# h3poteto/aws-global-accelerator-controller

Hardware: NVIDIA H100
Metric: objects reconciled/sec at 10^6 Service+Ingress; change-set bit-exact vs Go ref (higher is better)
Workload: dtype u8/u32 (bytes and indices)

## Files before the change

aws-global-accelerator-controller_b200/csrc/gar_pipeline.h:

```cpp
#pragma once

#include <stdio.h>
#include <stdlib.h>

#include <initializer_list>

#include "gar_rows.h"

#if defined(__CUDA_ARCH__)
#define GAR_ATOMIC_ADD(p, v) atomicAdd((p), (v))
#else
#define GAR_ATOMIC_ADD(p, v) (*(p) += (v))
#endif


enum Slot {
  S_DERIVED, S_OFLAGS, S_OKEY_HASH, S_STAGE_GA, S_STAGE_R53, S_ANN_R53, S_ANN_NAME, S_ANN_TAGS, S_ANN_LISTEN, S_DPORT_BEGIN, S_DPORTS,
  S_TOK_CODE, S_TOK_NAME, S_TOK_REGION,
  S_ACC_FLAGS, S_ACC_OWNER_KEY, S_ACC_OWNER, S_ACC_THOST, S_ACC_MANAGED, S_ACC_OWNER_HASH, S_ACC_THOST_HASH, S_REC_NAME_HASH, S_VAL_KEY_HASH,
  S_REC_ZONE, S_VAL_REC, S_VAL_CLS, S_VAL_KEY, S_VAL_ORPHAN, S_VAL_LINK, S_ACC_DIGEST,
  S_R53_MODE, S_R53_ACC, S_R53_ACC_DNS, S_PAIR_BEGIN, S_PAIR_OBJ, S_PAIR_HN, S_PAIR_CODE, S_PAIR_ZONE, S_PAIR_REC,
  S_IX_LB, S_IX_OWNER = S_IX_LB + 3, S_IX_THOST = S_IX_OWNER + 3, S_IX_ZONE = S_IX_THOST + 3, S_IX_VAL = S_IX_ZONE + 3,
  S_IX_ALIAS = S_IX_VAL + 3, S_IX_OBJ = S_IX_ALIAS + 3, S_IX_OVN = S_IX_OBJ + 3,
  S_SORT_KEYS = S_IX_OVN + 3, S_SORT_VALS, S_SORT_KEYS_ALT, S_SORT_VALS_ALT, S_SORT_TAGS,
  S_COUNTS, S_STATUS_GA, S_STATUS_R53, S_OPS, S_ERRFLAG, S_IX_EG, S_IX_EG_ENT, S_IX_EG_PAD,
  S_VAL_OBJ, S_ACC_OBJ, S_OBJ_CANON, S_OWN_BEGIN, S_OWN_FILL, S_OWN_ENT, S_OWN_MULTI,
  S_IXA_BEGIN, S_IXA_FILL, S_IXA_ENT, S_IXA_MULTI, S_OVN_FILL, S_OVN_MULTI, S_LB_HASH, S_REC_FLAGS, S_LBI_RES,
  S_NSLOTS
};


struct FClassify {
  DevTables T;
  Work W;
  u32 *derived_public;
  u8 *oflags;
  u32 *errflag;
  GAR_HD void operator()(u32 i) const {
    classify_object(T, W, i);
    W.obj_canon[i] = i;
    u32 dv = W.derived[i];
    if (dv & OBJ_KEY_BAD) GAR_ATOMIC_ADD(errflag, 1u);
    derived_public[i] = dv & 0xFFu;
  }
};
struct FTokenise {
  DevTables T;
  Work W;
  static constexpr int kStageCols = 1;
  static constexpr u32 kStageBytes = 24 * 1024;
  static constexpr bool kStageByDefault = true;
  GAR_HD void operator()(u32 i) const { tokenise_hostname(T, W, i); }
  GAR_HD const u8 *stage_slab(int) const { return T.o.slab; }
  GAR_HD bool stage_window(int, u32 r0, u32 r1, u64 *lo, u64 *hi) const {
    gar_str a = T.o.lbi_hostname[r0], b = T.o.lbi_hostname[r1 - 1];
    *lo = GAR_STR_OFF(a);
    *hi = GAR_STR_OFF(b) + GAR_STR_LEN(b);
    return true;
  }
  template <class View>
  GAR_HD void run(u32 i, const View &view) const { tokenise_hostname_at(T, W, i, view(0, T.o.lbi_hostname[i])); }
};
struct FDigestAccel {
  DevTables T;
  Work W;
  GAR_HD void operator()(u32 i) const { digest_accelerator(T, W, i); }
};
struct FExpand {
  const u32 *begin;
  u32 nparents;
  u32 *parent_of;
  GAR_HD void operator()(u32 c) const {
    u32 lo = 0, hi = nparents;
    while (hi - lo > 1) {
      u32 mid = (lo + hi) >> 1;
      if (begin[mid] <= c) lo = mid;
      else hi = mid;
    }
    parent_of[c] = lo;
  }
// ... 58 lines not shown
  }
};
constexpr u32 BIG_BLOCKS = 528;
struct FClassifyBigRecords {
  DevTables T;
  Work W;
  const u32 *big, *huge;
  GAR_HD void operator()(u32 i) const {
    const u32 blk = i >> 8, tid = i & 255u, nbig = big[0], nhuge = huge[0];
    for (u32 k = blk; k < nbig; k += BIG_BLOCKS) {
      u32 r = big[1 + k];
      for (u32 v = T.a.rec_val_begin[r] + tid; v < T.a.rec_val_begin[r + 1]; v += 256) {
        W.val_rec[v] = r;
        classify_value(T, W, v);
      }
    }
    for (u32 k = 0; k < nhuge; k++) {
      u32 r = huge[1 + k];
      for (u32 v = T.a.rec_val_begin[r] + i; v < T.a.rec_val_begin[r + 1]; v += BIG_BLOCKS * 256) {
        W.val_rec[v] = r;
        classify_value(T, W, v);
      }
    }
  }
};
struct FJsonCount {
  DevTables T;
  Work W;
  GAR_HD void operator()(u32 i) const {
    u32 n = 0;
    if (W.derived[i] & GAR_DV_PORTS_FROM_ANN) {
      u32 stk[GAR_JSON_STACK_WORDS];
      int c = json_listen_ports(mkstr(T.o.slab, W.ann_listen[i]), nullptr, stk);
      n = c < 0 ? 0u : (u32)c;
    }
    W.dport_begin[i] = n;
  }
};
struct FJsonWrite {
  DevTables T;
  Work W;
  GAR_HD void operator()(u32 i) const {
    if (!(W.derived[i] & GAR_DV_PORTS_FROM_ANN)) return;
    if (W.dport_begin[i + 1] == W.dport_begin[i] || W.dport_begin[i + 1] > W.dport_cap) return;
    u32 stk[GAR_JSON_STACK_WORDS];
    json_listen_ports(mkstr(T.o.slab, W.ann_listen[i]), W.dports + W.dport_begin[i], stk);
  }
};

struct FLbHash {
  DevTables T;
  Work W;
  GAR_HD void operator()(u32 i) const {
    u64 h = key_hash_lb(mkstr(T.a.slab, T.a.lb_region[i]), mkstr(T.a.slab, T.a.lb_name[i]));
    W.lb_hash[i] = h;
    ix_count(W.hist[IX_LB], h);
  }
};
struct FRowLb {
  DevTables T;
  Work W;
  GAR_HD bool make(u32 i, u64 *h, IdxEntry *e) const {
    *h = W.lb_hash[i];
    e->a0 = T.a.lb_state[i];
    e->a1 = 0;
    e->s0 = T.a.lb_name[i];
    e->s1 = T.a.lb_region[i];
    return true;
  }
};
struct FRowOwner {
  DevTables T;
  Work W;
  GAR_HD bool make(u32 i, u64 *h, IdxEntry *e) const {
    u32 fl = W.acc_flags[i];
    *h = W.acc_owner_hash[i];
    e->a0 = fl;
    e->a1 = 0;
    e->s0 = W.acc_owner_key[i];
    e->s1 = 0;
    return (fl & ACC_MINE) && (fl & ACC_OWNER_KEYED) && i < W.acc_guest_from;
  }
};
struct FRowThost {
  DevTables T;
  Work W;
  GAR_HD bool make(u32 i, u64 *h, IdxEntry *e) const {
    *h = W.acc_thost_hash[i];
    e->a0 = e->a1 = 0;
    e->s0 = W.acc_thost[i];
    e->s1 = T.a.acc_dns[i];
    return (W.acc_flags[i] & ACC_MINE) != 0 && (!W.sharded || i >= W.acc_guest_from);
  }
};
struct FRowZone {
  DevTables T;
  GAR_HD bool make(u32 i, u64 *h, IdxEntry *e) const {
    Str zn = mkstr(T.a.slab, T.a.zone_name[i]);
    bool valid = zn.n >= 1 && zn.p[zn.n - 1] == '.';
    *h = valid ? key_hash_str(substr(zn, 0, zn.n - 1)) : 0;
    e->a0 = e->a1 = 0;
    e->s0 = T.a.zone_name[i];
    e->s1 = 0;
    return valid;
  }
};
struct FZoneLenMask {
  DevTables T;
  Work W;
  unsigned long long *mask;
  GAR_HD void operator()(u32 z) const {
    Str zn = mkstr(T.a.slab, T.a.zone_name[z]);
    if (zn.n < 1 || zn.p[zn.n - 1] != '.') return;
    ix_count(W.hist[IX_ZONE], key_hash_str(substr(zn, 0, zn.n - 1)));
    u32 b = zn.n - 1 < 255 ? zn.n - 1 : 255;
#if defined(__CUDA_ARCH__)
    atomicOr(&mask[b >> 6], 1ull << (b & 63));
#else
    mask[b >> 6] |= 1ull << (b & 63);
#endif
// ... 596 lines not shown
    return HashIdx{begin, ent, nb - 1};
  }

  bool prepared = false;
  u64 n_dports = 0;
  u32 *errflag = nullptr;

  u32 acc_guest_from = 0xFFFFFFFFu;
  u32 sharded = 0;
  bool orphan_sweep = true;
  bool allow_empty_cache = false;

  void alloc_obj_work() {
    const u32 n = T.o.n_objects, nlbi = T.o.n_lbi;
    W.derived = (u32 *)be.ensure(S_DERIVED, 4 * (size_t)(n + 1));
    W.okey_hash = (u64 *)be.ensure(S_OKEY_HASH, 8 * (size_t)(n + 1));
    W.ann_r53 = (gar_str *)be.ensure(S_ANN_R53, 8 * (size_t)(n + 1));
    W.ann_name = (gar_str *)be.ensure(S_ANN_NAME, 8 * (size_t)(n + 1));
    W.ann_tags = (gar_str *)be.ensure(S_ANN_TAGS, 8 * (size_t)(n + 1));
    W.ann_listen = (gar_str *)be.ensure(S_ANN_LISTEN, 8 * (size_t)(n + 1));
    W.dport_begin = (u32 *)be.out_dport_begin(n);
    W.tok_code = (u8 *)be.out_tok_code(nlbi);
    W.tok_name = (gar_str *)be.out_tok_name(nlbi);
    W.tok_region = (gar_str *)be.out_tok_region(nlbi);
    W.lbi_res = (LbiRes *)be.ensure(S_LBI_RES, sizeof(LbiRes) * (size_t)(nlbi + 1));
    W.r53_mode = (u8 *)be.ensure(S_R53_MODE, (size_t)n + 1);
    W.r53_acc = (u32 *)be.ensure(S_R53_ACC, 4 * (size_t)(n + 1));
    W.r53_acc_dns = (gar_str *)be.ensure(S_R53_ACC_DNS, 8 * (size_t)(n + 1));
    W.obj_canon = (u32 *)be.ensure(S_OBJ_CANON, 4 * (size_t)(n + 1));
  }
  CanonHook canon_hook(u32 b0, u32 b1) const { return CanonHook{W.obj_canon, T.o.slab, b0, b1}; }
  void alloc_work() {
    const u32 nacc = T.a.n_accels, nrec = T.a.n_records, nval = T.a.n_values;
    alloc_obj_work();
    W.acc_flags = (u32 *)be.ensure(S_ACC_FLAGS, 4 * (size_t)(nacc + 1));
    W.acc_owner_key = (gar_str *)be.ensure(S_ACC_OWNER_KEY, 8 * (size_t)(nacc + 1));
    W.acc_owner = (gar_str *)be.ensure(S_ACC_OWNER, 8 * (size_t)(nacc + 1));
    W.acc_thost = (gar_str *)be.ensure(S_ACC_THOST, 8 * (size_t)(nacc + 1));
    W.acc_managed = (gar_str *)be.ensure(S_ACC_MANAGED, 8 * (size_t)(nacc + 1));
    W.acc_owner_hash = (u64 *)be.ensure(S_ACC_OWNER_HASH, 8 * (size_t)(nacc + 1));
    W.acc_thost_hash = (u64 *)be.ensure(S_ACC_THOST_HASH, 8 * (size_t)(nacc + 1));
    W.rec_name_hash = (u64 *)be.ensure(S_REC_NAME_HASH, 8 * (size_t)(nrec + 1));
    W.val_key_hash = (u64 *)be.ensure(S_VAL_KEY_HASH, 8 * (size_t)(nval + 1));
    W.rec_zone = (u32 *)be.ensure(S_REC_ZONE, 4 * (size_t)(nrec + 1));
    W.val_rec = (u32 *)be.ensure(S_VAL_REC, 4 * (size_t)(nval + 1));
    W.val_cls = (u8 *)be.ensure(S_VAL_CLS, nval + 1);
    W.val_key = (gar_str *)be.ensure(S_VAL_KEY, 8 * (size_t)(nval + 1));
    W.val_orphan = (u8 *)be.ensure(S_VAL_ORPHAN, nval + 1);
    W.val_obj = (u32 *)be.ensure(S_VAL_OBJ, 4 * (size_t)(nval + 1));
    W.acc_obj = (u32 *)be.ensure(S_ACC_OBJ, 4 * (size_t)(nacc + 1));
    W.val_link = (ValLink *)be.ensure(S_VAL_LINK, sizeof(ValLink) * (size_t)(nval + 1));
    W.acc_digest = (AccDigest *)be.ensure(S_ACC_DIGEST, sizeof(AccDigest) * (size_t)(nacc + 1));
    W.lb_hash = (u64 *)be.ensure(S_LB_HASH, 8 * (size_t)(T.a.n_lbs + 1));
    W.rec_flags = (u8 *)be.ensure(S_REC_FLAGS, (size_t)nrec + 1);
    for (int k = 0; k < IX_N; k++) W.hist[k] = IxHist{nullptr, 0};
    W.pair_cap = 0;
    W.dport_cap = 0;
    errflag = (u32 *)be.ensure(S_ERRFLAG, 256);
    be.fill32(errflag, 0, FW_WORDS);
    W.acc_guest_from = acc_guest_from;
    W.sharded = sharded;
  }
  void stage1() {
    const u32 n = T.o.n_objects, nlbi = T.o.n_lbi, nacc = T.a.n_accels, nrec = T.a.n_records, nval = T.a.n_values;
    u32 *derived_public = (u32 *)be.out_derived(n);
    if (n) be.for_each("classify_objects", n, FClassify{T, W, derived_public, nullptr, errflag});
    if (nlbi) be.for_each_staged("tokenise_hostnames", nlbi, FTokenise{T, W});
    if (nacc) be.for_each("digest_accelerators", nacc, FDigestAccel{T, W});
    if (T.a.n_lbs) be.for_each("hash_load_balancers", T.a.n_lbs, FLbHash{T, W});
    {
      unsigned long long *zm = (unsigned long long *)(errflag + 16 + 8);
      be.fill32((u32 *)zm, 0, 8);
      if (T.a.n_zones) be.for_each("zone_len_mask", T.a.n_zones, FZoneLenMask{T, W, zm});
      W.zone_len_mask = (const u64 *)zm;
    }
    if (nrec) {
      u32 *big = (u32 *)be.ensure(S_SORT_KEYS, 4 * (size_t)(nval / REC_INLINE_VALUES + 2));
      u32 *huge = (u32 *)be.ensure(S_SORT_VALS, 4 * (size_t)(nval / REC_HUGE_VALUES + 2));
      be.fill32(big, 0, 1);
      be.fill32(huge, 0, 1);
      be.for_each_staged("prepare_records", nrec, FPrepareRecord{T, W, big, huge});
      if (nval > REC_INLINE_VALUES) be.for_each("prepare_records", BIG_BLOCKS * 256, FClassifyBigRecords{T, W, big, huge});
    }
  }
  struct IxPlan {
    u32 off[IX_N] = {}, nb[IX_N] = {}, rows[IX_N] = {};
    bool want[IX_N] = {};
    u32 total_nb = 0;
    u64 total_rows = 0;
  };
  IxPlan planA;
  u32 *ixa_begin = nullptr, *ixa_fill = nullptr, *ixa_multi = nullptr;
  IdxEntry *ixa_ent = nullptr;
  u32 ovn_nb = 0;
  void arm_group_a(u32 want_mask) {
    const u32 rows[IX_N] = {T.a.n_lbs, T.a.n_accels, T.a.n_accels, T.a.n_zones, T.a.n_values, T.a.n_records, T.o.n_objects, 0};
    const u32 load[IX_N] = {1, 1, 1, 1, 1, 2, 1, 8};
    planA = IxPlan{};
    for (int k = 0; k < IX_OVN; k++) {
      planA.want[k] = (want_mask >> k) & 1u;
      if (!planA.want[k]) continue;
      planA.rows[k] = rows[k];
      planA.nb[k] = next_pow2(rows[k] / load[k] < 16 ? 16 : rows[k] / load[k]);
      planA.off[k] = planA.total_nb;
      planA.total_nb += planA.nb[k];
      planA.total_rows += rows[k];
    }
    ixa_begin = (u32 *)be.ensure(S_IXA_BEGIN, 4 * (size_t)(planA.total_nb + 2));
    be.fill32(ixa_begin, 0, (size_t)planA.total_nb + 2);
    for (int k = 0; k < IX_OVN; k++)
      if (planA.want[k]) W.hist[k] = IxHist{ixa_begin + planA.off[k], planA.nb[k] - 1};
  }
  HashIdx group_a_index(int k) const { return HashIdx{ixa_begin + planA.off[k], ixa_ent, planA.nb[k] - 1}; }
  template <class RowF>
  FIdxPlaceDirect<RowF> placer(int k, RowF rowf) const {
    return FIdxPlaceDirect<RowF>{rowf, ixa_fill + planA.off[k], ixa_ent, planA.nb[k] - 1};
  }
  void finish_group_a() {
    u32 *overflow = errflag + FW_IDX_OVERFLOW;
    be.exclusive_scan(ixa_begin, planA.total_nb + 1);
    ixa_fill = (u32 *)be.ensure(S_IXA_FILL, 4 * (size_t)(planA.total_nb + 1));
    ixa_ent = (IdxEntry *)be.ensure(S_IXA_ENT, sizeof(IdxEntry) * (size_t)(planA.total_rows + 1));
    const u32 multi_cap = (u32)(planA.total_rows / 2 + 1);
    ixa_multi = (u32 *)be.ensure(S_IXA_MULTI, 4 * (size_t)(multi_cap + 2));
    be.copy32(ixa_fill, ixa_begin, (size_t)planA.total_nb + 1);
    be.fill32(ixa_multi, 0, 1);
    const IxPlan &P = planA;
    auto n = [&](int k) { return P.want[k] ? P.rows[k] : 0u; };
    be.for_each_multi("idx_place", {n(IX_LB), n(IX_THOST), n(IX_ZONE), n(IX_ALIAS), n(IX_OBJ), P.total_nb},
                      placer(IX_LB, FRowLb{T, W}), placer(IX_THOST, FRowThost{T, W}), placer(IX_ZONE, FRowZone{T}),
                      placer(IX_ALIAS, FRowAlias{T, W}), placer(IX_OBJ, FRowObj{T, W}), FIdxMultiList{ixa_begin, ixa_multi});
    const CanonHook canon = P.want[IX_OBJ] ? canon_hook(P.off[IX_OBJ], P.off[IX_OBJ] + P.nb[IX_OBJ]) : CanonHook{};
    be.for_each_dyn("idx_order", ixa_multi, multi_cap, FIdxOrderMulti{ixa_begin, ixa_ent, ixa_multi, overflow, canon});
    if (P.want[IX_LB]) W.ix_lb = group_a_index(IX_LB);
    if (P.want[IX_THOST]) W.ix_thost = group_a_index(IX_THOST);
    if (P.want[IX_ZONE]) W.ix_zone = group_a_index(IX_ZONE);
    if (P.want[IX_ALIAS]) W.ix_alias = group_a_index(IX_ALIAS);
    if (P.want[IX_OBJ]) W.ix_obj = group_a_index(IX_OBJ);
  }
  void resolve_owners(bool link_aliases) {
    const u32 n = T.o.n_objects, nacc = T.a.n_accels, nval = T.a.n_values, nseg = 2 * n;
    u32 *overflow = errflag + FW_IDX_OVERFLOW;
    W.own_begin = (u32 *)be.ensure(S_OWN_BEGIN, 4 * (size_t)(nseg + 2));
    be.fill32(W.own_begin, 0, (size_t)nseg + 1);
    u32 *ovn = nullptr;
    if (!force_radix) {
      ovn_nb = next_pow2(nval / 8 < 16 ? 16 : nval / 8);
      ovn = (u32 *)be.ensure(S_IX_OVN + 0, 4 * (size_t)(ovn_nb + 2));
      be.fill32(ovn, 0, (size_t)ovn_nb + 2);
      W.hist[IX_OVN] = IxHist{ovn, ovn_nb - 1};
    } else {
      W.hist[IX_OVN] = IxHist{nullptr, 0};
    }
    const u32 nlbi = T.o.n_lbi;
    if (link_aliases) be.for_each_multi("value_joins", {nval, nacc, nlbi}, FValueJoins{T, W}, FResolveAccel{T, W}, FLbiResolve{T, W});
    else be.for_each_multi("resolve_owners", {nval, nacc, nlbi}, FResolveValue{T, W}, FResolveAccel{T, W}, FLbiResolve{T, W});
    be.exclusive_scan(W.own_begin, nseg + 1);
    IdxEntry *own = (IdxEntry *)be.ensure(S_OWN_ENT, sizeof(IdxEntry) * ((size_t)nacc + nval + 1));
    if (!force_radix) {
      be.exclusive_scan(ovn, ovn_nb + 1);
      u32 *ovn_cursor = (u32 *)be.ensure(S_OVN_FILL, 4 * (size_t)(ovn_nb + 1));
      IdxEntry *ovn_ent = (IdxEntry *)be.ensure(S_IX_OVN + 1, sizeof(IdxEntry) * (size_t)(nval + 1));
      u32 *ovn_multi = (u32 *)be.ensure(S_OVN_MULTI, 4 * (size_t)(nval / 2 + 3));
      u32 *own_cursor = (u32 *)be.ensure(S_OWN_FILL, 4 * (size_t)(nseg + 1));
      const u32 own_multi_cap = (u32)(((u64)nacc + nval) / 2 + 1);
      u32 *own_multi = (u32 *)be.ensure(S_OWN_MULTI, 4 * (size_t)(own_multi_cap + 2));
      be.copy32(ovn_cursor, ovn, (size_t)ovn_nb + 1);
      be.copy32(own_cursor, W.own_begin, (size_t)nseg + 1);
      be.fill32(ovn_multi, 0, 1);
      be.fill32(own_multi, 0, 1);
      be.for_each_multi("idx_place", {nval, ovn_nb, nacc, nval, nseg}, FIdxPlaceDirect<FRowOvn>{FRowOvn{T, W}, ovn_cursor, ovn_ent, ovn_nb - 1},
                        FIdxMultiList{ovn, ovn_multi}, FOwnPlace{T, W, own_cursor, own, 0}, FOwnPlace{T, W, own_cursor, own, nacc},
                        FIdxMultiList{W.own_begin, own_multi});
      be.for_each_dyn("idx_order", ovn_multi, nval / 2 + 1, FIdxOrderMulti{ovn, ovn_ent, ovn_multi, overflow});
      be.for_each_dyn("idx_order", own_multi, own_multi_cap, FIdxOrderMulti{W.own_begin, own, own_multi, overflow});
      W.ix_ovn = HashIdx{ovn, ovn_ent, ovn_nb - 1};
    } else {
      const u32 nx = nacc + nval;
      u32 *keys = (u32 *)be.ensure(S_SORT_KEYS, 4 * (size_t)(nx + 1));
      u32 *vals = (u32 *)be.ensure(S_SORT_VALS, 4 * (size_t)(nx + 1));
      u32 *keys2 = (u32 *)be.ensure(S_SORT_KEYS_ALT, 4 * (size_t)(nx + 1));
      u32 *vals2 = (u32 *)be.ensure(S_SORT_VALS_ALT, 4 * (size_t)(nx + 1));
      if (nx) {
        be.for_each("own_keys", nx, FOwnKeys{T, W, keys, vals});
        be.sort_pairs(keys, vals, keys2, vals2, nx, ilog2(nseg + 1) + 1);
        be.for_each("own_gather", nx, FOwnGather{T, W, vals, W.own_begin + nseg, own});
      }
      W.ix_ovn = build_index(S_IX_OVN, nval, 8, FRowOvn{T, W}, overflow, true);
    }
    W.own = own;
    owners_stale = false;
  }
  bool owner_indexes = false;
  void build_owner_indexes() {
    if (owner_indexes) return;
    u32 *overflow = errflag + FW_IDX_OVERFLOW;
    W.ix_owner = build_index(S_IX_OWNER, T.a.n_accels, 1, FRowOwner{T, W}, overflow, force_radix);
    W.ix_val = build_index(S_IX_VAL, T.a.n_values, 1, FRowVal{T, W}, overflow, force_radix);
    owner_indexes = true;
  }

  void prepare_route() {
    alloc_work();
    arm_group_a(1u << IX_ALIAS);
    stage1();
    finish_group_a();
  }
  void prepare_directory() {
    alloc_work();
// ... 415 lines not shown
```

aws-global-accelerator-controller_b200/csrc/gar_rows.h:

```cpp
#pragma once

#include "gar_common.h"
#include "gar_json.h"


struct DevTables {
  gar_objects o;
  gar_actual a;
  const u8 *cluster;
  u32 cluster_len;
};

enum {
  OBJ_HAS_NAME_ANN = 1u << 8,
  OBJ_HAS_TAGS_ANN = 1u << 9,
  OBJ_KEY_BAD = 1u << 10,
};

enum {
  ACC_MINE = 1u << 0,
  ACC_OWNER_KEYED = 1u << 1,
  ACC_OWNER_INGRESS = 1u << 2,
  ACC_OWNER_3PART = 1u << 3,
  ACC_HAS_MANAGED = 1u << 4, ACC_HAS_OWNER = 1u << 5, ACC_HAS_THOST = 1u << 6,
// ... 15 lines not shown
  u32 lis;
  u32 eg;
  u32 pr_begin;
  u32 ep_begin;
  u16 n_ports, n_eps;
  i32 port0, port1;
  gar_str name;
  gar_str thost;
  gar_str owner_key;
  gar_str ep0;
};
enum {
  ACCD_ENABLED = 1u << 8,
  ACCD_MANAGED_TRUE = 1u << 9,
  ACCD_LIS_NONE = 1u << 10, ACCD_LIS_MANY = 1u << 11,
  ACCD_LIS_UDP = 1u << 12,
  ACCD_EG_NONE = 1u << 13, ACCD_EG_MANY = 1u << 14,
};
struct alignas(16) ValLink {
  u32 alias_row, pad;
  gar_str alias_dns;
};
struct alignas(32) LbiRes {
  u32 lb;
  u32 acc;
  gar_str acc_dns;
  gar_str lb_dns;
  gar_str lb_arn;
};
enum { LBI_OK = 0, LBI_DNS_MISMATCH = 1, LBI_NOT_ACTIVE = 2, LBI_NOT_FOUND = 3 };
#define LBI_ROW_MASK 0x3FFFFFFFu
GAR_HD u32 lbi_verdict(const LbiRes &r) { return r.lb >> 30; }
GAR_HD u32 lbi_lb(const LbiRes &r) { return r.lb == GAR_NONE ? GAR_NONE : r.lb & LBI_ROW_MASK; }
GAR_HD u32 lbi_acc_count(const LbiRes &r) { return r.acc >> 30; }
GAR_HD u32 lbi_acc(const LbiRes &r) { return lbi_acc_count(r) ? r.acc & LBI_ROW_MASK : GAR_NONE; }

enum IxId { IX_LB, IX_OWNER, IX_THOST, IX_ZONE, IX_VAL, IX_ALIAS, IX_OBJ, IX_OVN, IX_N };
struct IxHist {
  u32 *cnt;
  u32 mask;
};
#if defined(__CUDA_ARCH__)
#define GAR_HIST_ADD(p) atomicAdd((p), 1u)
#else
#define GAR_HIST_ADD(p) (++*(p))
#endif
GAR_HD void ix_count(const IxHist &h, u64 key_hash) {
  if (h.cnt) GAR_HIST_ADD(&h.cnt[(u32)key_hash & h.mask]);
}

struct Work {
  IxHist hist[IX_N];
  u64 *lb_hash;
  u8 *rec_flags;
  u32 pair_cap;
  u32 dport_cap;
  u32 *derived;
  u64 *okey_hash;
  gar_str *ann_r53;
  gar_str *ann_name;
  gar_str *ann_tags;
  gar_str *ann_listen;
  u32 *dport_begin;
  i32 *dports;
  u8 *tok_code;
  gar_str *tok_name, *tok_region;
  LbiRes *lbi_res;
  u32 *acc_flags;
  gar_str *acc_owner_key;
  gar_str *acc_owner;
  gar_str *acc_thost;
  gar_str *acc_managed;
  AccDigest *acc_digest;
  u64 *acc_owner_hash;
  u64 *acc_thost_hash;
  u32 *rec_zone;
  u64 *rec_name_hash;
  u32 *val_rec;
  u8 *val_cls;
  gar_str *val_key;
  u64 *val_key_hash;
  u8 *val_orphan;
  ValLink *val_link;
  u32 acc_guest_from;
  u32 sharded;
  u32 *val_obj;
  u32 *acc_obj;
  u32 *obj_canon;
  u32 *own_begin;
  const IdxEntry *own;
  u8 *r53_mode;
  u32 *r53_acc;
  gar_str *r53_acc_dns;
  u32 *pair_begin;
  u32 *pair_obj;
  gar_str *pair_hn;
  u8 *pair_code;
  u32 *pair_zone;
  u32 *pair_rec;
  HashIdx ix_lb;
  HashIdx ix_owner;
  HashIdx ix_thost;
  HashIdx ix_zone;
  const u64 *zone_len_mask;
  HashIdx ix_val;
  HashIdx ix_alias;
// ... 244 lines not shown
      d.ep_begin = A.eg_ep_begin[eb];
      u32 ne = A.eg_ep_begin[eb + 1] - d.ep_begin;
      d.n_eps = (u16)(ne > 0xFFFF ? 0xFFFF : ne);
      if (ne > 0) d.ep0 = A.ep_id[d.ep_begin];
    }
  }
  d.name = A.acc_name[a];
  d.thost = thost;
  d.owner_key = key;
  W.acc_digest[a] = d;
  const u64 owner_hash = (fl & ACC_OWNER_KEYED) ? key_hash_kinded((fl & ACC_OWNER_INGRESS) ? 1u : 0u, mkstr(A.slab, key)) : 0;
  const u64 thost_hash = (fl & ACC_MINE) ? gar_hash(mkstr(A.slab, thost)) : 0;
  W.acc_owner_hash[a] = owner_hash;
  W.acc_thost_hash[a] = thost_hash;
  if (acc_in_owner_index(W, a, fl)) ix_count(W.hist[IX_OWNER], owner_hash);
  if (acc_in_thost_index(W, a, fl)) ix_count(W.hist[IX_THOST], thost_hash);
  W.acc_flags[a] = fl;
  W.acc_owner_key[a] = key;
  W.acc_owner[a] = owner;
  W.acc_thost[a] = thost;
  W.acc_managed[a] = managed;
}


#define R53_HERITAGE "\"heritage=aws-global-accelerator-controller,cluster="

GAR_HD void classify_value_at(const DevTables &T, const Work &W, u32 v, Str s) {
  const gar_actual &A = T.a;
  gar_str ref = A.val_value[v];
  u8 cls = VAL_NOT_OWNER;
  gar_str key = 0;
  const u32 hl = (u32)(sizeof(R53_HERITAGE) - 1);
  u32 fixed = hl + T.cluster_len + 1 + 8 + 1;
  if (s.n >= fixed && HAS_PREFIX_LIT(s, R53_HERITAGE) && streq(substr(s, hl, T.cluster_len), Str{T.cluster, T.cluster_len}) &&
      s.p[hl + T.cluster_len] == ',' && s.p[s.n - 1] == '"') {
    u32 ro = hl + T.cluster_len + 1;
    Str rest = substr(s, ro, s.n - 1 - ro);
    if (HAS_PREFIX_LIT(rest, "service/")) cls = VAL_OWNER_SERVICE;
    else if (HAS_PREFIX_LIT(rest, "ingress/")) cls = VAL_OWNER_INGRESS;
    if (cls) {
      key = GAR_STR(GAR_STR_OFF(ref) + ro + 8, rest.n - 8);
      if (count_slashes(substr(rest, 8, rest.n - 8)) == 1) cls |= VAL_OWNER_3PART;
    }
  }
  W.val_cls[v] = cls;
  W.val_key[v] = key;
  const u64 vkh = cls ? key_hash_kinded((cls & VAL_OWNER_INGRESS) ? 1u : 0u, substr(s, (u32)(GAR_STR_OFF(key) - GAR_STR_OFF(ref)), (u32)GAR_STR_LEN(key))) : 0;
  W.val_key_hash[v] = vkh;
  if (cls) ix_count(W.hist[IX_VAL], vkh);
}
GAR_HD void classify_value(const DevTables &T, const Work &W, u32 v) { classify_value_at(T, W, v, mkstr(T.a.slab, T.a.val_value[v])); }


template <class C>
GAR_HD u32 lb_walk(const DevTables &T, const Work &W, C &c, Str region, Str name, u32 *state) {
  IdxEntry e;
  while (idx_next(W.ix_lb, c, &e))
    if (streq(mkstr(T.a.slab, e.s0), name) && streq(mkstr(T.a.slab, e.s1), region)) {
      *state = e.a0;
      return e.row;
    }
  return GAR_NONE;
}
GAR_HD u32 find_lb(const DevTables &T, const Work &W, Str region, Str name, u32 *state) {
  Cursor c = idx_open(W.ix_lb, key_hash_lb(region, name));
  return lb_walk(T, W, c, region, name, state);
}

struct OwnRange {
  u32 pos, end;
};
GAR_HD OwnRange own_accs(const Work &W, u32 i) {
  const u32 s = 2 * W.obj_canon[i];
  return OwnRange{W.own_begin[s], W.own_begin[s + 1]};
}
GAR_HD OwnRange own_vals(const Work &W, u32 i) {
  const u32 s = 2 * W.obj_canon[i] + 1;
  return OwnRange{W.own_begin[s], W.own_begin[s + 1]};
}

struct OwnerIter {
  Cursor c;
  Str key;
};
GAR_HD OwnerIter owner_open(const Work &W, u64 key_hash, Str key) { return OwnerIter{idx_open(W.ix_owner, key_hash), key}; }
GAR_HD bool owner_match(const DevTables &T, const IdxEntry &e, u32 kind, Str key) {
  return ((((e.a0 & ACC_OWNER_INGRESS) != 0) ? 1u : 0u) == kind) && streq(mkstr(T.a.slab, e.s0), key);
}
GAR_HD u32 owner_next(const DevTables &T, const Work &W, u32 kind, OwnerIter &it) {
  IdxEntry e;
  while (idx_next(W.ix_owner, it.c, &e))
    if (owner_match(T, e, kind, it.key)) return e.row;
  return GAR_NONE;
}

template <class C>
GAR_HD u32 thost_walk(const DevTables &T, const Work &W, C &c, Str hostname, u32 *first, gar_str *first_dns, u32 *second = nullptr) {
  u32 n = 0;
  *first = GAR_NONE;
  if (second) *second = GAR_NONE;
  IdxEntry e;
  while (idx_next(W.ix_thost, c, &e)) {
    if (!streq(mkstr(T.a.slab, e.s0), hostname)) continue;
    if (n == 0) {
      *first = e.row;
      *first_dns = e.s1;
    } else if (second) {
      *second = e.row;
    }
    if (++n >= 2) break;
  }
  return n;
}
GAR_HD u32 find_by_hostname(const DevTables &T, const Work &W, Str hostname, u32 *first, gar_str *first_dns, u32 *second = nullptr) {
  Cursor c = idx_open(W.ix_thost, key_hash_str(hostname));
  return thost_walk(T, W, c, hostname, first, first_dns, second);
}

GAR_HD void lbi_resolve(const DevTables &T, const Work &W, u32 r) {
  if (W.tok_code[r] > GAR_TOK_NLB) return;
  const gar_actual &A = T.a;
  const Str host = mkstr(T.o.slab, T.o.lbi_hostname[r]);
  const Str region = mkstr(T.o.slab, W.tok_region[r]), name = mkstr(T.o.slab, W.tok_name[r]);
  PreCursor cl = idx_open_pre(W.ix_lb, key_hash_lb(region, name)), ch = idx_open_pre(W.ix_thost, key_hash_str(host));
  LbiRes res;
  u32 state = 0;
  const u32 lb = lb_walk(T, W, cl, region, name, &state);
  res.lb_dns = lb != GAR_NONE ? A.lb_dns[lb] : 0;
  res.lb_arn = lb != GAR_NONE ? A.lb_arn[lb] : 0;
  u32 acc = GAR_NONE;
  res.acc_dns = 0;
  const u32 nacc = thost_walk(T, W, ch, host, &acc, &res.acc_dns);
  res.acc = (nacc << 30) | (acc & LBI_ROW_MASK);
  res.lb = GAR_NONE;
  if (lb != GAR_NONE) {
    const u32 v = !streq(mkstr(A.slab, res.lb_dns), host) ? LBI_DNS_MISMATCH : state != GAR_LB_ACTIVE ? LBI_NOT_ACTIVE : LBI_OK;
    res.lb = (v << 30) | lb;
  }
  W.lbi_res[r] = res;
}

GAR_HD bool zone_len_possible(const Work &W, u32 n) {
  u32 b = n < 255 ? n : 255;
  return (W.zone_len_mask[b >> 6] >> (b & 63)) & 1ull;
}
GAR_HD u32 find_hosted_zone(const DevTables &T, const Work &W, Str hostname) {
  Str t = hostname;
  for (;;) {
    if (t.n == 0) return GAR_NONE;
    if (zone_len_possible(W, t.n)) {
      Cursor c = idx_open(W.ix_zone, key_hash_str(t));
      IdxEntry e;
      while (idx_next(W.ix_zone, c, &e)) {
        Str zn = mkstr(T.a.slab, e.s0);
        if (zn.n == t.n + 1 && streq(substr(zn, 0, t.n), t)) return e.row;
      }
    }
    u32 k = find_byte(t, 0, '.');
    if (k >= t.n) return GAR_NONE;
    t = substr(t, k + 1, t.n - k - 1);
  }
}

GAR_HD bool record_name_matches(Str name, Str hostname) {
  u32 w = GAR_NONE;
  for (u32 k = find_byte(name, 0, '\\'); k + 4 <= name.n; k = find_byte(name, k + 1, '\\'))
    if (name.p[k + 1] == '0' && name.p[k + 2] == '5' && name.p[k + 3] == '2') {
      w = k;
      break;
    }
  if (w == GAR_NONE) return name.n == hostname.n + 1 && name.p[name.n - 1] == '.' && streq(substr(name, 0, hostname.n), hostname);
  if (name.n - 3 != hostname.n + 1) return false;
  if (name.p[name.n - 1] != '.') return false;
  if (w >= hostname.n || hostname.p[w] != '*') return false;
  if (!streq(substr(name, 0, w), substr(hostname, 0, w))) return false;
  u32 tail = hostname.n - w - 1;
  return streq(substr(name, w + 4, tail), substr(hostname, w + 1, tail));
}


GAR_HD Cursor cursor_none() { return Cursor{0, 0, 0}; }
GAR_HD Cursor u_open(const HashIdx &ix, bool active, u64 h) { return active ? idx_open(ix, h) : cursor_none(); }

GAR_HD bool u_bucket_step(const HashIdx &ix, bool searching, Cursor &c, IdxEntry *e) {
  bool step = searching && c.pos < c.end;
  if (step) {
    *e = load_entry(ix.ent + c.pos++);
    return e->tag == c.tag;
  }
  return false;
// ... 924 lines not shown
  W.val_orphan[v] = orphan;
}

GAR_HD void r53_orphan_alias(const DevTables &T, const Work &W, u32 r, OpSink &s) {
  const gar_actual &A = T.a;
  if (!A.rec_has_alias[r]) return;
  u32 zone = W.rec_zone[r];
  Str name = mkstr(A.slab, A.rec_name[r]);
  u64 h = key_hash_zoned_h(zone, W.rec_name_hash[r]);
  Cursor c = idx_open(W.ix_ovn, h);
  IdxEntry e;
  while (idx_next(W.ix_ovn, c, &e)) {
    if (e.a1 != zone || !streq(mkstr(A.slab, e.s0), name)) continue;
    Str val = mkstr(A.slab, e.s1);
    bool dup = false;
    Cursor c2 = idx_open(W.ix_ovn, h);
    IdxEntry e2;
    while (idx_next(W.ix_ovn, c2, &e2) && e2.row < e.row) {
      if (e2.a1 == zone && streq(mkstr(A.slab, e2.s0), name) && streq(mkstr(A.slab, e2.s1), val)) {
        dup = true;
        break;
      }
    }
    if (dup) continue;
    s.put(GAR_OP_HEAD(GAR_OP_R53_DELETE_RECORD, GAR_CTRL_R53, 0), GAR_NONE, 0, zone, r, e.row);
  }
}


struct DevBindings {
  gar_bindings b;
  HashIdx ix_eg;
};

GAR_HD bool egb_eg_exists(const DevBindings &B, Str arn) {
  Cursor c = idx_open(B.ix_eg, gar_hash(arn));
  IdxEntry e;
  while (idx_next(B.ix_eg, c, &e))
    if (streq(mkstr(B.b.slab, e.s0), arn)) return true;
  return false;
}

GAR_HD u32 egb_lb_of(const DevTables &T, const Work &W, u32 lbi_row, u32 *detail) {
  u32 code = W.tok_code[lbi_row];
  *detail = 0;
  if (code == GAR_TOK_NOT_AWS || code == GAR_TOK_PANIC) {
    *detail = GAR_D_NOT_ELB;
    return GAR_NONE;
  }
  if (code >= GAR_TOK_ERR_NOT_ELB) {
    *detail = GAR_D_NOT_ELB + (code - GAR_TOK_ERR_NOT_ELB);
    return GAR_NONE;
  }
  u32 st;
  u32 lb = find_lb(T, W, mkstr(T.o.slab, W.tok_region[lbi_row]), mkstr(T.o.slab, W.tok_name[lbi_row]), &st);
  if (lb == GAR_NONE) *detail = GAR_D_LB_NOT_FOUND;
  return lb;
}

GAR_HD u32 egb_reconcile(const DevTables &T, const Work &W, const DevBindings &B, u32 k, OpSink &s) {
  const gar_bindings &b = B.b;
  const gar_actual &A = T.a;
  u32 flags = b.egb_flags[k];
  u32 eb = b.egb_ep_begin[k], n = b.egb_ep_begin[k + 1] - eb;
  Str eg_arn = mkstr(b.slab, b.egb_eg_arn[k]);
  auto H = [](u32 op) { return GAR_OP_HEAD(op, GAR_CTRL_EGB, 0); };
  if (flags & GAR_EGB_DELETING) {
    if (n == 0 || !egb_eg_exists(B, eg_arn)) {
      s.put(H(GAR_OP_EGB_REMOVE_FINALIZER), k, 0, GAR_NONE, GAR_NONE, GAR_NONE);
      return GAR_STATUS(GAR_ST_OK, 0, 0);
    }
    u32 len = n;
    for (u32 i = 0; i < n; i++) {
      u32 src = 2 * i < n - 1 ? 2 * i : n - 1;
      s.put(H(GAR_OP_EGB_REMOVE_ENDPOINT), k, 0, eb + src, GAR_NONE, GAR_NONE);
      if (i + 1 > len) return GAR_STATUS(GAR_ST_PANIC, 0, 0);
      len--;
    }
    s.put(H(GAR_OP_EGB_UPDATE_STATUS), k, 0, GAR_NONE, GAR_NONE, GAR_NONE);
    return GAR_STATUS(GAR_ST_REQUEUE_1S, 0, 0);
  }
  if (!(flags & GAR_EGB_HAS_FINALIZERS)) {
    s.put(H(GAR_OP_EGB_ADD_FINALIZER), k, 0, GAR_NONE, GAR_NONE, GAR_NONE);
    return GAR_STATUS(GAR_ST_OK, 0, 0);
  }
  u32 jb = 0, nj = 0;
  u32 refkind = b.egb_ref_kind[k];
  if (refkind != GAR_EGB_REF_NONE) {
    u32 kind = refkind == GAR_EGB_REF_SERVICE ? GAR_KIND_SERVICE : GAR_KIND_INGRESS;
    Str key = mkstr(b.slab, b.egb_ref_key[k]);
    Cursor c = idx_open(W.ix_obj, key_hash_kinded(kind, key));
    IdxEntry e;
    u32 obj = GAR_NONE;
    while (idx_next(W.ix_obj, c, &e))
      if (e.a0 == kind && streq(mkstr(T.o.slab, e.s0), key)) {
        obj = e.row;
        break;
      }
    if (obj == GAR_NONE) return GAR_STATUS(GAR_ST_ERR_RETRY, GAR_D_REF_NOT_FOUND, 0);
    jb = T.o.obj_lbi_begin[obj];
    nj = T.o.obj_lbi_begin[obj + 1] - jb;
  }
  for (u32 j = 0; j < nj; j++) {
    u32 detail;
    if (egb_lb_of(T, W, jb + j, &detail) == GAR_NONE) return GAR_STATUS(GAR_ST_ERR_RETRY, detail, 0);
  }
  auto arn_of = [&](u32 j) {
    u32 d;
// ... 19 lines not shown
  for (u32 j = 0; j < nj; j++)
    if (is_first(j) && !in_status(arn_of(j))) nnew++;
  for (u32 x = 0; x < n; x++)
    if (!in_arns(mkstr(b.slab, b.ep_id[eb + x]))) nrem++;
  if (nnew == 0 && nrem == 0 && (flags & GAR_EGB_OBSERVED)) return GAR_STATUS(GAR_ST_OK, 0, 0);
  if (!egb_eg_exists(B, eg_arn)) return GAR_STATUS(GAR_ST_ERR_RETRY, GAR_D_EG_NOT_FOUND, 0);
  if (nrem > 0 && nj == 0) return GAR_STATUS(GAR_ST_PANIC, 0, 0);
  for (u32 x = 0; x < n; x++)
    if (!in_arns(mkstr(b.slab, b.ep_id[eb + x]))) s.put(H(GAR_OP_EGB_REMOVE_ENDPOINT), k, 0, eb + x, GAR_NONE, GAR_NONE);
  Str last_region = nj ? mkstr(T.o.slab, W.tok_region[jb + nj - 1]) : Str{T.o.slab, 0};
  for (u32 j = 0; j < nj; j++) {
    if (!is_first(j) || in_status(arn_of(j))) continue;
    u32 jl = j;
    for (u32 i = j + 1; i < nj; i++)
      if (streq(arn_of(i), arn_of(j))) jl = i;
    u32 st;
    u32 lb2 = find_lb(T, W, last_region, mkstr(T.o.slab, W.tok_name[jb + jl]), &st);
    if (lb2 == GAR_NONE) return GAR_STATUS(GAR_ST_ERR_RETRY, GAR_D_LB_NOT_FOUND, 0);
    if (st != GAR_LB_ACTIVE) return GAR_STATUS(GAR_ST_REQUEUE_30S, 0, 0);
    s.put(H(GAR_OP_EGB_ADD_ENDPOINT), k, 0, lb2, GAR_NONE, GAR_NONE);
  }
  for (u32 j = 0; j < nj; j++)
    if (is_first(j)) {
      u32 d;
      s.put(H(GAR_OP_EGB_UPDATE_WEIGHT), k, 0, egb_lb_of(T, W, jb + j, &d), GAR_NONE, GAR_NONE);
    }
  s.put(H(GAR_OP_EGB_UPDATE_STATUS), k, 0, GAR_NONE, GAR_NONE, GAR_NONE);
  return GAR_STATUS(GAR_ST_OK, 0, 0);
}

enum { RS_LB = 0, RS_ACC = 1, RS_ZONE = 2, RS_MISS = 3, RS_N = 4 };
struct ReadSetBits {
  u32 *bits;
  u32 wb[RS_N + 1];
};
GAR_HD void rs_mark(const ReadSetBits &B, u32 s, u32 row) {
  const u32 b = B.wb[s] * 32 + row, m = 1u << (b & 31);
#if defined(__CUDA_ARCH__)
  u32 *w = B.bits + (b >> 5);
  if (!(__ldcg(w) & m)) atomicOr(w, m);
#else
  B.bits[b >> 5] |= m;
#endif
}
GAR_HD u32 read_set_row_items(const DevTables &T, const Work &W, u32 i) {
  const OwnRange a = own_accs(W, i), v = own_vals(W, i);
  return (T.o.obj_lbi_begin[i + 1] - T.o.obj_lbi_begin[i]) + (a.end - a.pos) + (v.end - v.pos) + 1;
}
GAR_HD void read_set_row_item(const DevTables &T, const Work &W, const ReadSetBits &B, u32 i, u32 q) {
  const u32 jb = T.o.obj_lbi_begin[i], nj = T.o.obj_lbi_begin[i + 1] - jb;
  if (q < nj) {
    const u32 p = jb + q;
    if (W.tok_code[p] > GAR_TOK_NLB) return;
    u32 st;
    const u32 lb = find_lb(T, W, mkstr(T.o.slab, W.tok_region[p]), mkstr(T.o.slab, W.tok_name[p]), &st);
    if (lb != GAR_NONE) rs_mark(B, RS_LB, lb);
    else rs_mark(B, RS_MISS, p);
    u32 a0, a1;
    gar_str dns;
    find_by_hostname(T, W, mkstr(T.o.slab, T.o.lbi_hostname[p]), &a0, &dns, &a1);
    if (a0 != GAR_NONE) rs_mark(B, RS_ACC, a0);
    if (a1 != GAR_NONE) rs_mark(B, RS_ACC, a1);
    return;
  }
  q -= nj;
  const OwnRange a = own_accs(W, i);
  if (q < a.end - a.pos) return rs_mark(B, RS_ACC, W.own[a.pos + q].row);
  q -= a.end - a.pos;
  const OwnRange v = own_vals(W, i);
  if (q < v.end - v.pos) return rs_mark(B, RS_ZONE, owned_hit(load_entry(W.own + v.pos + q)).zone);
  if (!(W.derived[i] & GAR_DV_R53_ANNOTATED)) return;
  const Str all = mkstr(T.o.slab, W.ann_r53[i]);
  u32 pos = 0;
  Str piece;
  while (next_piece(all, &pos, &piece)) {
    const u32 z = find_hosted_zone(T, W, piece);
    if (z != GAR_NONE) rs_mark(B, RS_ZONE, z);
  }
}
GAR_HD u32 read_set_deleted_items(const Work &W, u32 kind, Str key, Cursor *c) {
  const u64 h = key_hash_kinded(kind, key);
  c[0] = idx_open(W.ix_owner, h);
  c[1] = idx_open(W.ix_val, h);
  return (c[0].end - c[0].pos) + (c[1].end - c[1].pos);
}
GAR_HD void read_set_deleted_item(const DevTables &T, const Work &W, const ReadSetBits &B, u32 kind, Str key, const Cursor *c, u32 q) {
  const u32 no = c[0].end - c[0].pos;
  if (q < no) {
    const IdxEntry e = load_entry(W.ix_owner.ent + c[0].pos + q);
    if (e.tag == c[0].tag && owner_match(T, e, kind, key)) rs_mark(B, RS_ACC, e.row);
    return;
  }
  const IdxEntry e = load_entry(W.ix_val.ent + c[1].pos + (q - no));
  if (e.tag == c[1].tag && owned_match(T, e, kind, key)) rs_mark(B, RS_ZONE, owned_hit(e).zone);
}
```

aws-global-accelerator-controller_b200/csrc/gar_shard.h:

```cpp
#pragma once

#include "gar_pipeline.h"

#if defined(__CUDA_ARCH__)
#define GAR_ATOMIC_OR(p, v) atomicOr((p), (v))
#else
#define GAR_ATOMIC_OR(p, v) (*(p) |= (v))
#endif

constexpr int SH_MAX_RANKS = GAR_SHARD_MAX_RANKS;
constexpr int SH_MAX_SEGS = 2 * SH_MAX_RANKS;
enum ShLevel { L_OBJ, L_ANN, L_LBI, L_PORT, L_ACC, L_TAG, L_LIS, L_PR, L_EG, L_EP, L_REC, L_VAL, L_ZONE, L_LB, L_STUB, L_STUBTAG, L_PROBE, L_NLEVELS };
static_assert(2 * L_NLEVELS + 1 <= GAR_SHARD_META_WORDS, "meta row too small");
constexpr int SH_MAX_STR = 4, SH_MAX_U8 = 3, SH_MAX_U32 = 1, SH_MAX_CHILD = 3;
enum { SH_ARENA_PLAN = 0, SH_ARENA_DIR = 1, SH_ARENA_HOME = 2 };
constexpr u32 SH_DROP = 255;
constexpr u32 SH_FOLLOW = 254;

struct LevelSchema {
  int n_str, n_u8, n_u32, has_gid, n_child;
  int child[SH_MAX_CHILD];
};
static const LevelSchema SH_SCHEMA[L_NLEVELS] = {
     {2, 3, 1, 1, 3, {L_ANN, L_LBI, L_PORT}},
// ... 429 lines not shown
  GAR_HD void operator()(u32 i) const {
    u64 off = GAR_STR_OFF(key[i]), len = GAR_STR_LEN(key[i]), nl = ns_len[i];
    ns[i] = GAR_STR(off, nl);
    name[i] = GAR_STR(off + nl + 1, len - nl - 1);
  }
};
struct FShZoneBegin {
  const u32 *rec_zone;
  u32 n_rec;
  u32 *begin;
  GAR_HD void operator()(u32 z) const {
    u32 lo = 0, hi = n_rec;
    while (lo < hi) {
      u32 mid = (lo + hi) >> 1;
      if (rec_zone[mid] < z) lo = mid + 1;
      else hi = mid;
    }
    begin[z] = lo;
  }
};

struct FShZoneFingerprint {
  DevTables T;
  unsigned long long *acc;
  GAR_HD void operator()(u32 z) const {
    u64 h = hmix((u64)z + 1, gar_hash(mkstr(T.a.slab, T.a.zone_name[z])));
#if defined(__CUDA_ARCH__)
    atomicAdd(acc, (unsigned long long)h);
#else
    *acc += h;
#endif
  }
};
struct FShCheckZoneOrder {
  const u32 *rec_zone;
  u32 n_zones;
  u32 *bad;
  GAR_HD void operator()(u32 r) const {
    if (rec_zone[r] >= n_zones || (r > 0 && rec_zone[r - 1] > rec_zone[r])) GAR_ATOMIC_ADD(bad, 1u);
  }
};
constexpr int SH_META_ZONE_FP = 2 * L_NLEVELS;
#define GAR_E_SHARD_CONTRACT 2000


struct FShAnswer {
  DevTables T;
  Work W;
  const u32 *home;
  u32 *lb_mask, *stub_mask;
  GAR_HD void operator()(u32 p) const {
    const u32 bit = 1u << home[p];
    if (W.tok_code[p] <= GAR_TOK_NLB) {
      u32 st;
      u32 lb = find_lb(T, W, mkstr(T.o.slab, W.tok_region[p]), mkstr(T.o.slab, W.tok_name[p]), &st);
      if (lb != GAR_NONE && !(lb_mask[lb] & bit)) GAR_ATOMIC_OR(&lb_mask[lb], bit);
    }
    Str host = mkstr(T.o.slab, T.o.lbi_hostname[p]);
    Cursor c = idx_open(W.ix_thost, key_hash_str(host));
    IdxEntry e;
    u32 k = 0;
    while (k < 2 && idx_next(W.ix_thost, c, &e)) {
      if (!streq(mkstr(T.a.slab, e.s0), host)) continue;
      if (!(stub_mask[e.row] & bit)) GAR_ATOMIC_OR(&stub_mask[e.row], bit);
      k++;
    }
  }
};


struct ShGids {
  const u32 *obj, *lb, *acc, *lis, *eg, *rec, *val;
};
struct FShTranslateOps {
  gar_op *ops;
  ShGids g;
  GAR_HD u32 m(const u32 *tab, u32 v) const { return v >= GAR_PENDING ? v : tab[v]; }
  GAR_HD void operator()(u32 k) const {
    gar_op o = ops[k];
    o.obj = m(g.obj, o.obj);
    switch (o.head & 0xFFu) {
      case GAR_OP_GA_CREATE_CHAIN: o.a0 = m(g.lb, o.a0); break;
      case GAR_OP_GA_UPDATE_ACCEL: o.a0 = m(g.acc, o.a0); o.a1 = m(g.lb, o.a1); break;
      case GAR_OP_GA_CREATE_LISTENER: o.a0 = m(g.acc, o.a0); break;
      case GAR_OP_GA_UPDATE_LISTENER: o.a0 = m(g.acc, o.a0); o.a1 = m(g.lis, o.a1); break;
      case GAR_OP_GA_CREATE_EG: o.a0 = m(g.acc, o.a0); o.a1 = m(g.lis, o.a1); o.a2 = m(g.lb, o.a2); break;
      case GAR_OP_GA_UPDATE_EG: o.a0 = m(g.acc, o.a0); o.a1 = m(g.eg, o.a1); o.a2 = m(g.lb, o.a2); break;
      case GAR_OP_GA_DELETE_CHAIN: o.a0 = m(g.acc, o.a0); o.a1 = m(g.lis, o.a1); o.a2 = m(g.eg, o.a2); break;
      case GAR_OP_R53_CREATE: o.a1 = m(g.acc, o.a1); break;
      case GAR_OP_R53_UPSERT_A: o.a1 = m(g.acc, o.a1); o.a2 = m(g.rec, o.a2); break;
      case GAR_OP_R53_DELETE_RECORD: o.a1 = m(g.rec, o.a1); o.a2 = m(g.val, o.a2); break;
      default: break;
    }
    ops[k] = o;
  }
};


template <class B>
struct Sharder {
  B &be;
  gar_shard cfg{};
  u32 G = 1;
  DevTables S{};
  Pipeline<B> *slice_pipe = nullptr;
  Pipeline<B> *dir_pipe = nullptr;
  DevTables Dt{};
  const u32 *dir_home = nullptr, *dir_lb_gid = nullptr, *dir_stub_gid = nullptr;
// ... 496 lines not shown
```

Baseline: 189.6 million.

## Precompute LB DNS name/region positions to shortcut hash-index key matching

The LB hash pass now checks whether each load balancer's DNS name embeds its name and region at standard offsets, and stores the packed positions in a new per-LB array. The LB index rows store DNS and ARN plus a self flag, so a lookup whose hostname tokens sit at the same positions can match with a single DNS string compare. That one compare replaces separate name and region compares and the later DNS compare in lbi_resolve. It also reorders the multi-kernel launch to run LBI resolution first. The risk is extra work in the hash pass and possible correctness subtleties in the fast-path equivalence.

```diff
diff --git a/aws-global-accelerator-controller_b200/csrc/gar_pipeline.h b/aws-global-accelerator-controller_b200/csrc/gar_pipeline.h
--- a/aws-global-accelerator-controller_b200/csrc/gar_pipeline.h
+++ b/aws-global-accelerator-controller_b200/csrc/gar_pipeline.h
@@ -25,7 +25,7 @@
   S_SORT_KEYS = S_IX_OVN + 3, S_SORT_VALS, S_SORT_KEYS_ALT, S_SORT_VALS_ALT, S_SORT_TAGS,
   S_COUNTS, S_STATUS_GA, S_STATUS_R53, S_OPS, S_ERRFLAG, S_IX_EG, S_IX_EG_ENT, S_IX_EG_PAD,
   S_VAL_OBJ, S_ACC_OBJ, S_OBJ_CANON, S_OWN_BEGIN, S_OWN_FILL, S_OWN_ENT, S_OWN_MULTI,
-  S_IXA_BEGIN, S_IXA_FILL, S_IXA_ENT, S_IXA_MULTI, S_OVN_FILL, S_OVN_MULTI, S_LB_HASH, S_REC_FLAGS, S_LBI_RES,
+  S_IXA_BEGIN, S_IXA_FILL, S_IXA_ENT, S_IXA_MULTI, S_OVN_FILL, S_OVN_MULTI, S_LB_HASH, S_REC_FLAGS, S_LBI_RES, S_LB_DNS_POS,
   S_NSLOTS
 };
 
@@ -190,9 +190,19 @@
   DevTables T;
   Work W;
   GAR_HD void operator()(u32 i) const {
-    u64 h = key_hash_lb(mkstr(T.a.slab, T.a.lb_region[i]), mkstr(T.a.slab, T.a.lb_name[i]));
+    const gar_actual &A = T.a;
+    const Str region = mkstr(A.slab, A.lb_region[i]), name = mkstr(A.slab, A.lb_name[i]);
+    u64 h = key_hash_lb(region, name);
     W.lb_hash[i] = h;
     ix_count(W.hist[IX_LB], h);
+    const gar_str dns = A.lb_dns[i];
+    const Str d = mkstr(A.slab, dns);
+    const u32 pn = HAS_PREFIX_LIT(d, "internal-") ? 9 : 0, tail = region.n + (HAS_SUFFIX_LIT(d, ".elb.amazonaws.com") ? 18 : 14);
+    const u64 o = GAR_STR_OFF(dns);
+    u32 pos = GAR_NONE;
+    if (pn + name.n <= d.n && tail <= d.n && streq(substr(d, pn, name.n), name) && streq(substr(d, d.n - tail, region.n), region))
+      pos = dns_pos(o, GAR_STR(o + pn, name.n), GAR_STR(o + d.n - tail, region.n));
+    W.lb_dns_pos[i] = pos;
   }
 };
 struct FRowLb {
@@ -200,10 +210,11 @@
   Work W;
   GAR_HD bool make(u32 i, u64 *h, IdxEntry *e) const {
     *h = W.lb_hash[i];
-    e->a0 = T.a.lb_state[i];
-    e->a1 = 0;
-    e->s0 = T.a.lb_name[i];
-    e->s1 = T.a.lb_region[i];
+    const u32 pos = W.lb_dns_pos[i];
+    e->a0 = T.a.lb_state[i] | (pos != GAR_NONE ? LBD_SELF : 0u);
+    e->a1 = pos;
+    e->s0 = T.a.lb_dns[i];
+    e->s1 = T.a.lb_arn[i];
     return true;
   }
 };
@@ -906,6 +917,7 @@
     W.val_link = (ValLink *)be.ensure(S_VAL_LINK, sizeof(ValLink) * (size_t)(nval + 1));
     W.acc_digest = (AccDigest *)be.ensure(S_ACC_DIGEST, sizeof(AccDigest) * (size_t)(nacc + 1));
     W.lb_hash = (u64 *)be.ensure(S_LB_HASH, 8 * (size_t)(T.a.n_lbs + 1));
+    W.lb_dns_pos = (u32 *)be.ensure(S_LB_DNS_POS, 4 * (size_t)(T.a.n_lbs + 1));
     W.rec_flags = (u8 *)be.ensure(S_REC_FLAGS, (size_t)nrec + 1);
     for (int k = 0; k < IX_N; k++) W.hist[k] = IxHist{nullptr, 0};
     W.pair_cap = 0;
@@ -1007,8 +1019,8 @@
       W.hist[IX_OVN] = IxHist{nullptr, 0};
     }
     const u32 nlbi = T.o.n_lbi;
-    if (link_aliases) be.for_each_multi("value_joins", {nval, nacc, nlbi}, FValueJoins{T, W}, FResolveAccel{T, W}, FLbiResolve{T, W});
-    else be.for_each_multi("resolve_owners", {nval, nacc, nlbi}, FResolveValue{T, W}, FResolveAccel{T, W}, FLbiResolve{T, W});
+    if (link_aliases) be.for_each_multi("value_joins", {nlbi, nval, nacc}, FLbiResolve{T, W}, FValueJoins{T, W}, FResolveAccel{T, W});
+    else be.for_each_multi("resolve_owners", {nlbi, nval, nacc}, FLbiResolve{T, W}, FResolveValue{T, W}, FResolveAccel{T, W});
     be.exclusive_scan(W.own_begin, nseg + 1);
     IdxEntry *own = (IdxEntry *)be.ensure(S_OWN_ENT, sizeof(IdxEntry) * ((size_t)nacc + nval + 1));
     if (!force_radix) {
diff --git a/aws-global-accelerator-controller_b200/csrc/gar_rows.h b/aws-global-accelerator-controller_b200/csrc/gar_rows.h
--- a/aws-global-accelerator-controller_b200/csrc/gar_rows.h
+++ b/aws-global-accelerator-controller_b200/csrc/gar_rows.h
@@ -91,6 +91,7 @@
 struct Work {
   IxHist hist[IX_N];
   u64 *lb_hash;
+  u32 *lb_dns_pos;
   u8 *rec_flags;
   u32 pair_cap;
   u32 dport_cap;
@@ -441,19 +442,43 @@
 GAR_HD void classify_value(const DevTables &T, const Work &W, u32 v) { classify_value_at(T, W, v, mkstr(T.a.slab, T.a.val_value[v])); }
 
 
+GAR_HD u32 dns_pos(u64 base, gar_str name, gar_str region) {
+  const u64 pn = GAR_STR_OFF(name) - base, ln = GAR_STR_LEN(name), pr = GAR_STR_OFF(region) - base, lr = GAR_STR_LEN(region);
+  if (GAR_STR_OFF(name) < base || GAR_STR_OFF(region) < base || (pn | ln | pr | lr) > 255) return GAR_NONE;
+  return (u32)(pn | ln << 8 | pr << 16 | lr << 24);
+}
+#define LBD_SELF (1u << 8)
+struct LbHit {
+  u32 row;
+  u32 state;
+  gar_str dns;
+  gar_str arn;
+  bool dns_eq;
+};
 template <class C>
-GAR_HD u32 lb_walk(const DevTables &T, const Work &W, C &c, Str region, Str name, u32 *state) {
+GAR_HD LbHit lb_walk(const DevTables &T, const Work &W, C &c, Str region, Str name, const Str *host, u32 pos) {
+  const gar_actual &A = T.a;
   IdxEntry e;
-  while (idx_next(W.ix_lb, c, &e))
-    if (streq(mkstr(T.a.slab, e.s0), name) && streq(mkstr(T.a.slab, e.s1), region)) {
-      *state = e.a0;
-      return e.row;
-    }
-  return GAR_NONE;
-}
+  while (idx_next(W.ix_lb, c, &e)) {
+    const bool self = host && (e.a0 & LBD_SELF) && e.a1 == pos;
+    bool dns_eq = self && streq(mkstr(A.slab, e.s0), *host);
+    if (!dns_eq && !(streq(mkstr(A.slab, A.lb_name[e.row]), name) && streq(mkstr(A.slab, A.lb_region[e.row]), region))) continue;
+    if (host && !self) dns_eq = streq(mkstr(A.slab, e.s0), *host);
+    return LbHit{e.row, e.a0 & ~LBD_SELF, e.s0, e.s1, dns_eq};
+  }
+  return LbHit{GAR_NONE, 0, 0, 0, false};
+}
+GAR_HD u32 lbi_pos(const DevTables &T, const Work &W, u32 p) { return dns_pos(GAR_STR_OFF(T.o.lbi_hostname[p]), W.tok_name[p], W.tok_region[p]); }
 GAR_HD u32 find_lb(const DevTables &T, const Work &W, Str region, Str name, u32 *state) {
   Cursor c = idx_open(W.ix_lb, key_hash_lb(region, name));
-  return lb_walk(T, W, c, region, name, state);
+  const LbHit hit = lb_walk(T, W, c, region, name, nullptr, GAR_NONE);
+  *state = hit.state;
+  return hit.row;
+}
+GAR_HD LbHit find_lb_of_row(const DevTables &T, const Work &W, u32 p) {
+  const Str region = mkstr(T.o.slab, W.tok_region[p]), name = mkstr(T.o.slab, W.tok_name[p]), host = mkstr(T.o.slab, T.o.lbi_hostname[p]);
+  Cursor c = idx_open(W.ix_lb, key_hash_lb(region, name));
+  return lb_walk(T, W, c, region, name, &host, lbi_pos(T, W, p));
 }
 
 struct OwnRange {
@@ -508,23 +533,21 @@
 
 GAR_HD void lbi_resolve(const DevTables &T, const Work &W, u32 r) {
   if (W.tok_code[r] > GAR_TOK_NLB) return;
-  const gar_actual &A = T.a;
   const Str host = mkstr(T.o.slab, T.o.lbi_hostname[r]);
   const Str region = mkstr(T.o.slab, W.tok_region[r]), name = mkstr(T.o.slab, W.tok_name[r]);
   PreCursor cl = idx_open_pre(W.ix_lb, key_hash_lb(region, name)), ch = idx_open_pre(W.ix_thost, key_hash_str(host));
   LbiRes res;
-  u32 state = 0;
-  const u32 lb = lb_walk(T, W, cl, region, name, &state);
-  res.lb_dns = lb != GAR_NONE ? A.lb_dns[lb] : 0;
-  res.lb_arn = lb != GAR_NONE ? A.lb_arn[lb] : 0;
+  const LbHit lb = lb_walk(T, W, cl, region, name, &host, lbi_pos(T, W, r));
+  res.lb_dns = lb.dns;
+  res.lb_arn = lb.arn;
   u32 acc = GAR_NONE;
   res.acc_dns = 0;
   const u32 nacc = thost_walk(T, W, ch, host, &acc, &res.acc_dns);
   res.acc = (nacc << 30) | (acc & LBI_ROW_MASK);
   res.lb = GAR_NONE;
-  if (lb != GAR_NONE) {
-    const u32 v = !streq(mkstr(A.slab, res.lb_dns), host) ? LBI_DNS_MISMATCH : state != GAR_LB_ACTIVE ? LBI_NOT_ACTIVE : LBI_OK;
-    res.lb = (v << 30) | lb;
+  if (lb.row != GAR_NONE) {
+    const u32 v = !lb.dns_eq ? LBI_DNS_MISMATCH : lb.state != GAR_LB_ACTIVE ? LBI_NOT_ACTIVE : LBI_OK;
+    res.lb = (v << 30) | lb.row;
   }
   W.lbi_res[r] = res;
 }
@@ -1555,8 +1578,7 @@
     *detail = GAR_D_NOT_ELB + (code - GAR_TOK_ERR_NOT_ELB);
     return GAR_NONE;
   }
-  u32 st;
-  u32 lb = find_lb(T, W, mkstr(T.o.slab, W.tok_region[lbi_row]), mkstr(T.o.slab, W.tok_name[lbi_row]), &st);
+  const u32 lb = find_lb_of_row(T, W, lbi_row).row;
   if (lb == GAR_NONE) *detail = GAR_D_LB_NOT_FOUND;
   return lb;
 }
@@ -1682,8 +1704,7 @@
   if (q < nj) {
     const u32 p = jb + q;
     if (W.tok_code[p] > GAR_TOK_NLB) return;
-    u32 st;
-    const u32 lb = find_lb(T, W, mkstr(T.o.slab, W.tok_region[p]), mkstr(T.o.slab, W.tok_name[p]), &st);
+    const u32 lb = find_lb_of_row(T, W, p).row;
     if (lb != GAR_NONE) rs_mark(B, RS_LB, lb);
     else rs_mark(B, RS_MISS, p);
     u32 a0, a1;
diff --git a/aws-global-accelerator-controller_b200/csrc/gar_shard.h b/aws-global-accelerator-controller_b200/csrc/gar_shard.h
--- a/aws-global-accelerator-controller_b200/csrc/gar_shard.h
+++ b/aws-global-accelerator-controller_b200/csrc/gar_shard.h
@@ -505,8 +505,7 @@
   GAR_HD void operator()(u32 p) const {
     const u32 bit = 1u << home[p];
     if (W.tok_code[p] <= GAR_TOK_NLB) {
-      u32 st;
-      u32 lb = find_lb(T, W, mkstr(T.o.slab, W.tok_region[p]), mkstr(T.o.slab, W.tok_name[p]), &st);
+      const u32 lb = find_lb_of_row(T, W, p).row;
       if (lb != GAR_NONE && !(lb_mask[lb] & bit)) GAR_ATOMIC_OR(&lb_mask[lb], bit);
     }
     Str host = mkstr(T.o.slab, T.o.lbi_hostname[p]);
```

Measured after the change: 194.4 million (median of 6 runs). +2.5%, better.
